# VITA-Group/LightGaussian

Measured on AMD Instinct MI355X. Metric: views/sec fwd+bwd @1080p (N Gaussians), higher is better.
Workload: dtype f32; 1 GPU; 3000000 synthetic Gaussians (SURVEY 8d generator, seed 20250103), 1920x1080, SH degree 3, fwdbwd through gaussian_renderer.render, 200-camera orbit; n_gaussians=3000000, width=1920, height=1080, mode=fwdbwd, views=200, exp=hardware, loss=L1 (HIP, lg_loss_forward/backward with LG_FLAG_L1_ONLY), parallelism=camera-shard x1

## Files before the change

### lightgaussian_amd/csrc/lg_api.hip

```cpp
#include "lg_host.h"
#include "lg_wave.h"
#include "lg_rows.h"
#include "lg_preprocess.h"
#include "lg_binning.h"
#include "lg_blend.h"
#include "lg_loss.h"
#include "lg_prune.h"
#include "lg_knn.h"
#include "lg_compact.h"
#include "lg_vq.h"
#include "lg_vq_train.h"
#include "lg_vq_color.h"
#include "lg_vq_color_bwd.h"
#include "lg_adam.h"
#include "lg_densify.h"
#include "lg_mcmc.h"
#include "lg_features.h"
#include "lg_camera.h"
#include "lg_absgrad.h"
#include "lg_filter3d.h"
#include "lg_normals.h"
#include "lg_distortion.h"
#include "lg_sensitivity.h"
#include "lg_tsdf.h"
// ... 186 lines not shown
    const lg_view* v; const lg_gaussians* g; const Bounded* bounded; lg_alloc_fn alloc; void* alloc_user; int weight_policy;
    float* out_color; int32_t* out_radii; int32_t* out_count; float* out_score; void** binning_out; int64_t* num_rendered;
    hipStream_t stream; bool debug, prof;
    int N, nblk; ViewGeom q; GeomView geo; ImgView img; BinView bin;
    KeyPlan kp; ForwardPlan plan;
    int64_t cap;
    bool k1_cleared_sort;
    PinnedSlot vslot;
    uint32_t* device_status() const { return bounded ? bounded->status : nullptr; }
    int front_end();
    int binning();
    int blend();
    int score();
    int epilogue();
};

int Forward::front_end()
{
    const bool count = out_count != nullptr;
    if (bounded) {
        if (!bounded->binning || bounded->capacity <= 0 || bounded->capacity >= (1ll << 30) || !(bounded->max_depth > 0.2f))
            return fail(LG_ERR_INVALID_ARGUMENT, "lg_forward_bounded: binning buffer, 0 < max_rendered < 2^30 and max_depth > 0.2 required");
        kp = make_key_plan(q.ntiles, N, __builtin_bit_cast(uint32_t, bounded->max_depth), v->flags);
        cap = bounded->capacity;
        bin = carve_bin(bounded->binning, cap, q.W, q.H, q.S);
        if (N == 0) {
            HIP_TRY(lg_zero_async(geo.counters, 16, stream));
            if (bounded->status) HIP_TRY(lg_zero_async(bounded->status, 16, stream));
            HIP_TRY(lg_zero_async(bin.ranges, (size_t)q.ntiles * 8, stream));
        }
    }
    plan = make_forward_plan(v->flags, count, weight_policy, N, bounded ? cap : 1);
    const bool host_words = bounded && bounded->host_status;
    if (host_words) {
        if (!vslot.p) return fail(LG_ERR_ALLOC, "hipHostMalloc of the status slot failed");
        if (N > 0) { vslot.p[1] = vslot.p[2] = vslot.p[3] = 0u; __atomic_store_n(&vslot.p[0], LG_STATUS_PENDING, __ATOMIC_RELEASE); }
        else memset(vslot.p, 0, 16);
    }
    uint32_t* k1_clear = nullptr;
    uint32_t k1_nclear = 0;
    if (bounded && plan.live) {
        k1_clear = (uint32_t*)bin.sort_temp;
        k1_nclear = (uint32_t)(lg_sort_clear_bytes(lg_sort_layout((size_t)cap), (unsigned)kp.sort_passes()) / 4);
    }
    k1_cleared_sort = k1_clear != nullptr;
    if (N > 0) {
        {
            ProfScope ps(prof, "preprocess", stream);
            const bool direct = !(v->flags & LG_FLAG_K1_LDS), raw = v->flags & LG_FLAG_RAW_PARAMS;
            const size_t k1_dyn = (direct && g->shs && !g->colors_precomp && !plan.k1_skip_color) ? LG_K1_PAD_LDS : 0;
            preprocess_kernel(raw, direct, v->flags & LG_FLAG_ANTIALIAS)<<<nblk, LG_PP, k1_dyn, stream>>>(
                N, g->M, v->sh_degree, q.W, q.H, v->tanfovx, v->tanfovy, v->scale_modifier, v->prefiltered, plan.k1_skip_color ? 1 : 0, v->viewmatrix,
                v->projmatrix, v->campos, g->means3D, g->shs, g->shs_rest, g->colors_precomp, g->opacities, g->scales, g->rotations, g->cov3D_precomp, geo,
                out_radii, plan.k1_clears_count ? out_count : nullptr, out_score, k1_clear, k1_nclear, (v->flags & LG_FLAG_SAVE_SH_JACOBIAN) ? 1 : 0);
        }
        KCHECK("lg_preprocess");
        {
            ProfScope ps(prof, "scan", stream);
            lg_scan_blocks<<<(nblk + LG_PART - 1) / LG_PART, LG_PART, 0, stream>>>(nblk, geo.blk_sum, geo.blk_dmax, geo.blk_off, geo.part_sum,
                                                                                  geo.part_dmax, geo.part_prefix, geo.counters + 8,
                                                                                  bounded ? (uint32_t)cap : 0xFFFFFFFFu,
                                                                                  bounded ? kp.depth_bits : 32, geo.counters,
                                                                                  host_words ? vslot.p : device_status());
        }
        KCHECK("lg_scan_blocks");
    }
    if (!bounded) {
        uint32_t h_counters[4] = {0, 0, 0, 0};
        if (N > 0) {
            PinnedSlot slot;
            if (!slot.p) return fail(LG_ERR_ALLOC, "hipHostMalloc of the read-back slot failed");
            HIP_TRY(hipMemcpyAsync(slot.p, geo.counters, 16, hipMemcpyDeviceToHost, stream));
            HIP_TRY(hipStreamSynchronize(stream));
            for (int k = 0; k < 4; k++) h_counters[k] = slot.p[k];
            if (v->prefiltered && h_counters[1]) return fail(LG_ERR_PREFILTERED, "Point is filtered although prefiltered is set. This shouldn't happen!");
            if (h_counters[0] & 1u) return fail(LG_ERR_INVALID_ARGUMENT, "more than 2^32-1 tile instances in one view");
        }
        cap = h_counters[3];
        if (cap >= (1ll << 30)) return fail(LG_ERR_INVALID_ARGUMENT, "more than 2^30-1 tile instances in one view");
        kp = make_key_plan(q.ntiles, N, h_counters[2], v->flags);
        plan = make_forward_plan(v->flags, count, weight_policy, N, cap);
        void* bin_p = alloc(alloc_user, carve_bin(nullptr, cap, q.W, q.H, q.S).total);
        if (!bin_p) return fail(LG_ERR_ALLOC, "binning allocator returned NULL");
        if (binning_out) *binning_out = bin_p;
        bin = carve_bin(bin_p, cap, q.W, q.H, q.S);
        if (num_rendered) *num_rendered = cap;
        if (cap == 0) HIP_TRY(lg_zero_async(bin.ranges, (size_t)q.ntiles * 8, stream));
    }
    g_stats.num_rendered = bounded ? -1 : cap;
    g_stats.num_visible = -1;
    return LG_OK;
}

int Forward::binning()
{
    if (!plan.live) return LG_OK;
    const int sort_begin = kp.sort_begin(), sort_end = kp.sort_end();
    const LgSortLayout SL = lg_sort_layout((size_t)cap);
    if (!k1_cleared_sort) HIP_TRY(lg_zero_async(bin.sort_temp, lg_sort_clear_bytes(SL, (unsigned)kp.sort_passes()), stream));
    uint32_t* hist = (uint32_t*)((char*)bin.sort_temp + SL.hist_off);
    {
        ProfScope ps(prof, "duplicate", stream);
        const int dgrid = std::max(1, std::min((nblk + 4 * LG_DUP_WAVES - 1) / (4 * LG_DUP_WAVES), LG_DUP_GRID));
        lg_duplicate<<<dgrid, LG_DUP_THREADS, 0, stream>>>(N, nblk, q.gx, kp.stored(), kp.store_drop, kp.gid_bits, sort_begin, sort_end, (uint32_t)cap, geo.touched,
                                                          geo.blk_off, geo.part_prefix, geo.counters, geo.offsets, geo.tinfo, bin.keys_in, q.ntiles, bin.ranges, hist,
                                                          kp.two_stage ? 0xFFFFFFFFu : 0u, bin.long_tiles);
    }
// ... 2180 lines not shown
```

### lightgaussian_amd/csrc/lg_binning.h

```cpp
#pragma once

#include "lg_host.h"
#include "lg_wave.h"

#define LG_PART 1024

__global__ void __launch_bounds__(LG_PART)
lg_scan_blocks(int nblk, const uint32_t* __restrict__ blk_sum, const uint32_t* __restrict__ blk_dmax, uint32_t* __restrict__ blk_off,
               uint32_t* part_sum, uint32_t* part_dmax, uint32_t* __restrict__ part_prefix, uint32_t* done, uint32_t capacity,
               int depth_bits, uint32_t* __restrict__ counters, uint32_t* __restrict__ status)
{
    __shared__ uint32_t wsum[16], wmax[16], wflag[16];
    __shared__ uint32_t s_last;
    const uint32_t tid = threadIdx.x, lane = tid & 63u, wave = tid >> 6;
    const int nparts = (int)gridDim.x;
    {
        const int i = (int)blockIdx.x * LG_PART + (int)tid;
        const uint32_t v = i < nblk ? blk_sum[i] : 0u, d = i < nblk ? blk_dmax[i] : 0u;
        const uint32_t inc = lg_wave_scan_incl(v, lane);
        uint32_t m = d & 0x7FFFFFFFu, f = d >> 31;
#pragma unroll
        for (int sh = 32; sh > 0; sh >>= 1) { m = max(m, (uint32_t)__shfl_xor((int)m, sh)); f |= (uint32_t)__shfl_xor((int)f, sh); }
        lg_block_scan_put(wsum, wave, lane, inc);
        if (lane == 63u) { wmax[wave] = m; wflag[wave] = f; }
// ... 63 lines not shown
}

#define LG_DUP_THREADS 1024
#ifndef LG_DUP_GRID
#define LG_DUP_GRID 512
#endif
#define LG_DUP_WAVES (LG_DUP_THREADS / 64)
__global__ void __launch_bounds__(LG_DUP_THREADS)
lg_duplicate(int N, int nblk, int gx, int stored_depth_bits, int store_drop, int gid_bits, int sort_begin, int sort_end, uint32_t capacity,
             const uint32_t* __restrict__ touched, const uint32_t* __restrict__ blk_off, const uint32_t* __restrict__ part_prefix,
             const uint32_t* __restrict__ counters,
             uint32_t* __restrict__ offsets, uint4* __restrict__ tinfo, uint64_t* __restrict__ keys,
             int ntiles, uint2* __restrict__ ranges, uint32_t* __restrict__ hist, uint32_t range_init, uint32_t* __restrict__ long_tiles)
{
    __shared__ uint32_t lh[LG_SORT_MAX_PASSES * 256];
    __shared__ uint32_t s_exc[LG_DUP_WAVES][64], s_xy[LG_DUP_WAVES][64], s_w[LG_DUP_WAVES][64], s_hi[LG_DUP_WAVES][64], s_lo[LG_DUP_WAVES][64];
    const uint32_t tid = threadIdx.x, lane = tid & 63u, wave = tid >> 6;
    for (int t = blockIdx.x * LG_DUP_THREADS + (int)tid; t < ntiles; t += gridDim.x * LG_DUP_THREADS) ranges[t] = make_uint2(range_init, 0u);
    if (blockIdx.x == 0 && tid == 0) long_tiles[0] = 0u;
    const int passes = (sort_end - sort_begin + 7) / 8;
    for (int i = (int)tid; i < passes * 256; i += LG_DUP_THREADS) lh[i] = 0;
    __syncthreads();
    if (counters[0] != 0u) return;
    const int sh = stored_depth_bits + gid_bits;
    const int ngroups = (nblk + 3) / 4;
    for (int g = blockIdx.x * LG_DUP_WAVES + (int)wave; g < ngroups; g += gridDim.x * LG_DUP_WAVES) {
        uint32_t t4[4], base4[4];
        uint4 r4[4];
#pragma unroll
        for (int u = 0; u < 4; u++) {
            const int b = g * 4 + u, i = b * 64 + (int)lane;
            t4[u] = (b < nblk && i < N) ? touched[i] : 0u;
            base4[u] = b < nblk ? blk_off[b] + part_prefix[b / LG_PART] : 0u;
        }
#pragma unroll
        for (int u = 0; u < 4; u++) {
            const int i = (g * 4 + u) * 64 + (int)lane;
            r4[u] = make_uint4(0, 0, 0, 0);
            if (t4[u]) r4[u] = tinfo[i];
        }
#pragma unroll
        for (int u = 0; u < 4; u++) {
            const int b = g * 4 + u, i = b * 64 + (int)lane;
            const uint32_t t = t4[u], base = base4[u];
            const uint4 r = r4[u];
            const uint32_t inc = lg_wave_scan_incl(t, lane);
            const uint32_t total = (uint32_t)__builtin_amdgcn_readlane((int)inc, 63);
            if (b < nblk && i < N) offsets[i] = base + inc;
            if (total != 0u) {
                const uint32_t exc = inc - t;
                if (t) tinfo[i].w = base + exc;
                s_exc[wave][lane] = exc;
                s_xy[wave][lane] = r.x;
                s_w[wave][lane] = (r.y & 0xFFFFu) - (r.x & 0xFFFFu);
                const uint64_t low = ((uint64_t)((r.z - LG_DEPTH_BIAS) >> store_drop) << gid_bits) | (uint32_t)i;
                s_lo[wave][lane] = (uint32_t)low;
                s_hi[wave][lane] = (uint32_t)(low >> 32);
                lg_wave_lds_sync();
                for (uint32_t p = lane; p < total; p += 64u) {
                    uint32_t j = 0;
#pragma unroll
                    for (uint32_t step = 32; step > 0; step >>= 1)
                        if (s_exc[wave][j + step] <= p) j += step;
                    const uint32_t k = p - s_exc[wave][j], w = s_w[wave][j], xy = s_xy[wave][j];
                    const uint32_t ky = k / w, kx = k - ky * w;
                    const uint32_t tile = ((xy >> 16) + ky) * (uint32_t)gx + (xy & 0xFFFFu) + kx;
                    const uint64_t pos = (uint64_t)base + p;
                    const uint64_t key = ((uint64_t)tile << sh) | ((uint64_t)s_hi[wave][j] << 32) | s_lo[wave][j];
                    if (pos < capacity) keys[pos] = key;
                    for (int q = 0; q < passes; q++) {
                        const int bit = sort_begin + 8 * q, nb = min(8, sort_end - bit);
                        atomicAdd(&lh[q * 256 + (uint32_t)((key >> bit) & ((1u << nb) - 1u))], 1u);
                    }
                }
                __builtin_amdgcn_wave_barrier();
            }
        }
    }
    __syncthreads();
    for (int i = (int)tid; i < passes * 256; i += LG_DUP_THREADS)
        if (lh[i]) atomicAdd(&hist[i], lh[i]);
}

__device__ __forceinline__ uint32_t lg_slot_of(const uint4 r, int tx, int ty)
{
    const int x0 = r.x & 0xFFFF, y0 = r.x >> 16, x1 = r.y & 0xFFFF;
    return r.w + (uint32_t)((ty - y0) * (x1 - x0) + (tx - x0));
}

#define LG_RUN_SHORT 32u
__device__ __forceinline__ uint32_t lg_low_bits(uint64_t key, int gid_bits, uint32_t gid_mask, int store_drop, uint32_t low_mask,
                                                const uint4* __restrict__ tinfo)
{
    if (store_drop == 0) return (uint32_t)(key >> gid_bits) & low_mask;
    return (tinfo[(uint32_t)key & gid_mask].z - LG_DEPTH_BIAS) & low_mask;
}

__device__ __forceinline__ void lg_wave_sort_run(uint32_t i, uint32_t e, int low_bits, int gid_bits, uint32_t gid_mask, int store_drop,
                                                 uint64_t* entries, uint64_t* scratch, const uint4* __restrict__ tinfo, uint32_t* cnt ,
                                                 uint32_t lane)
{
    const uint32_t low_mask = low_bits >= 32 ? 0xFFFFFFFFu : ((1u << low_bits) - 1u);
    uint64_t* src = entries;
    uint64_t* dst = scratch;
    for (int shift = 0; shift < low_bits; shift += 8) {
        const uint32_t dmask = (1u << min(8, low_bits - shift)) - 1u;
        for (uint32_t c = lane; c < 256u; c += 64u) cnt[c] = 0u;
        lg_wave_lds_sync();
        for (uint32_t a = i + lane; a < e; a += 64u)
            atomicAdd(&cnt[(lg_low_bits(src[a], gid_bits, gid_mask, store_drop, low_mask, tinfo) >> shift) & dmask], 1u);
        lg_wave_lds_sync();
        {
            const uint32_t c0 = cnt[4u * lane], c1 = cnt[4u * lane + 1u], c2 = cnt[4u * lane + 2u], c3 = cnt[4u * lane + 3u];
            const uint32_t own = c0 + c1 + c2 + c3;
            const uint32_t ex = lg_wave_scan_incl(own, lane) - own;
            cnt[4u * lane] = ex; cnt[4u * lane + 1u] = ex + c0; cnt[4u * lane + 2u] = ex + c0 + c1; cnt[4u * lane + 3u] = ex + c0 + c1 + c2;
        }
        lg_wave_lds_sync();
        for (uint32_t a0 = i; a0 < e; a0 += 64u) {
            const uint32_t a = a0 + lane;
            const bool valid = a < e;
            const uint64_t k = valid ? src[a] : 0ull;
            const uint32_t d = valid ? (lg_low_bits(k, gid_bits, gid_mask, store_drop, low_mask, tinfo) >> shift) & dmask : 0u;
            uint64_t peers = __ballot(valid);
#pragma unroll
            for (int b = 0; b < 8; b++) {
                const bool bit = (d >> b) & 1u;
                const uint64_t m = __ballot(bit);
                peers &= bit ? m : ~m;
            }
            const uint32_t below = prefix_popc(peers);
            uint32_t pos = 0;
            if (valid) pos = cnt[d] + below;
            lg_wave_lds_sync();
            if (valid && below == 0u) cnt[d] += (uint32_t)__popcll(peers);
            lg_wave_lds_sync();
            if (valid) dst[i + pos] = k;
        }
        __threadfence();
        uint64_t* t = src; src = dst; dst = t;
// ... 483 lines not shown
```

### lightgaussian_amd/csrc/lg_math.h

```cpp
#pragma once
#include <math.h>
#include <stddef.h>
#include <stdint.h>

#if defined(__HIPCC__)
#define LG_HD __host__ __device__ __forceinline__
#else
#define LG_HD static inline
#endif

#define LG_TILE 16
#define LG_ALPHA_MIN (1.0f / 255.0f)
#define LG_T_MIN 0.0001f
#define LG_ALPHA_MAX 0.99f

enum { LG_W_ONE = 0, LG_W_OPACITY = 1, LG_W_ALPHA = 2, LG_W_ALPHA_T = 3 };

LG_HD float lg_bits2f(uint32_t u) { union { uint32_t u; float f; } c; c.u = u; return c.f; }
LG_HD uint32_t lg_f2bits(float f) { union { uint32_t u; float f; } c; c.f = f; return c.u; }

LG_HD float lg_exp(float x)
{
    x = fmaxf(x, -87.0f);
    float t = x * 1.44269504088896341f;
// ... 110 lines not shown
    float b = o.U[0] * T2[3] + o.U[1] * T2[4] + o.U[2] * T2[5];
    float c = o.V[0] * T2[3] + o.V[1] * T2[4] + o.V[2] * T2[5];
    o.a = a + 0.3f; o.b = b; o.c = c + 0.3f;
    o.a0 = a; o.c0 = c;
}

#define LG_AA_FLOOR 0.000025f
LG_HD float lg_aa_ratio(float a0, float b, float c0, float a, float c)
{
    const float det0 = a0 * c0 - b * b;
    const float det1 = a * c - b * b;
    return det0 / det1;
}
LG_HD float lg_aa_rho(float x) { return sqrtf(fmaxf(LG_AA_FLOOR, x)); }
LG_HD float lg_aa_backward(float a0, float b, float c0, float a, float c, float op, float gp, float& dL_da, float& dL_db, float& dL_dc)
{
    const float det0 = a0 * c0 - b * b;
    const float det1 = a * c - b * b;
    const float x = det0 / det1;
    const float rho = lg_aa_rho(x);
    if (x > LG_AA_FLOOR) {
        const float gx = (op * gp) * 0.5f / rho;
        const float s = gx / (det1 * det1);
        const float bb = b * b;
        dL_da += s * (0.3f * (c0 * c + bb));
        dL_dc += s * (0.3f * (a0 * a + bb));
        dL_db += s * (-2.0f * b * (0.3f * (a0 + c0) + 0.09f));
    }
    return rho;
}

LG_HD void lg_view_point(const float* vm, float px, float py, float pz, float& vx, float& vy, float& vz)
{
    vx = vm[0] * px + vm[4] * py + vm[8] * pz + vm[12];
    vy = vm[1] * px + vm[5] * py + vm[9] * pz + vm[13];
    vz = vm[2] * px + vm[6] * py + vm[10] * pz + vm[14];
}
LG_HD void lg_hom_point(const float* pm, float px, float py, float pz, float& hx, float& hy, float& m_w)
{
    hx = pm[0] * px + pm[4] * py + pm[8] * pz + pm[12];
    hy = pm[1] * px + pm[5] * py + pm[9] * pz + pm[13];
    const float hw = pm[3] * px + pm[7] * py + pm[11] * pz + pm[15];
    m_w = 1.0f / (hw + 0.0000001f);
}
LG_HD void lg_focal(int W, int H, float tanfovx, float tanfovy, float& fx, float& fy)
{
    fx = (float)W / (2.0f * tanfovx); fy = (float)H / (2.0f * tanfovy);
}

struct LgSplat {
    float x, y, depth;
    float ha, nb, hc;
    float hx, hy;
    int radius;
    int rx0, ry0, rx1, ry1;
    int tx0, ty0, tx1, ty1;
};

template <bool AA>
LG_HD bool lg_project_t(const float* vm, const float* pm, float px, float py, float pz, const float* cov3D, float opacity,
                        int W, int H, float tanfovx, float tanfovy, LgSplat& o, float& op_out)
{
    float vx, vy, vz;
    lg_view_point(vm, px, py, pz, vx, vy, vz);
    if (vz <= 0.2f) return false;
    float hxm = pm[0] * px + pm[4] * py + pm[8] * pz + pm[12];
    float hym = pm[1] * px + pm[5] * py + pm[9] * pz + pm[13];
    float hwm = pm[3] * px + pm[7] * py + pm[11] * pz + pm[15];
    float p_w = 1.0f / (hwm + 0.0000001f);
    float ndcx = hxm * p_w, ndcy = hym * p_w;

    float fx, fy;
    lg_focal(W, H, tanfovx, tanfovy, fx, fy);
    LgEwa e;
    lg_ewa(vm, vx, vy, vz, fx, fy, 1.3f * tanfovx, 1.3f * tanfovy, e);
    LgCov2D c2;
    lg_cov2d(e.T2, cov3D, c2);
    const float a = c2.a, b = c2.b, c = c2.c;
    float det = a * c - b * b;
    if (det == 0.0f) return false;
    if (AA) { opacity = opacity * lg_aa_rho(lg_aa_ratio(c2.a0, b, c2.c0, a, c)); op_out = opacity; }
    float det_inv = 1.0f / det;
    float A = c * det_inv, B = -b * det_inv, C = a * det_inv;
    float mid = 0.5f * (a + c);
    float sq = sqrtf(fmaxf(0.1f, mid * mid - det));
    float l1 = mid + sq, l2 = mid - sq;
    float rad = ceilf(3.0f * sqrtf(fmaxf(l1, l2)));
    float ix = ((ndcx + 1.0f) * (float)W - 1.0f) * 0.5f;
    float iy = ((ndcy + 1.0f) * (float)H - 1.0f) * 0.5f;
    const int gx = (W + LG_TILE - 1) / LG_TILE, gy = (H + LG_TILE - 1) / LG_TILE;
    const float big = 1.0e7f;
    int r0 = (int)fminf(big, fmaxf(-big, (ix - rad) / (float)LG_TILE));
    int r1 = (int)fminf(big, fmaxf(-big, (iy - rad) / (float)LG_TILE));
    int r2 = (int)fminf(big, fmaxf(-big, (ix + rad + (float)(LG_TILE - 1)) / (float)LG_TILE));
    int r3 = (int)fminf(big, fmaxf(-big, (iy + rad + (float)(LG_TILE - 1)) / (float)LG_TILE));
    o.rx0 = r0 < 0 ? 0 : (r0 > gx ? gx : r0);
    o.ry0 = r1 < 0 ? 0 : (r1 > gy ? gy : r1);
    o.rx1 = r2 < 0 ? 0 : (r2 > gx ? gx : r2);
    o.ry1 = r3 < 0 ? 0 : (r3 > gy ? gy : r3);
    if ((o.rx1 - o.rx0) * (o.ry1 - o.ry0) == 0) return false;
    o.x = ix; o.y = iy; o.depth = vz; o.radius = (int)rad;
    o.ha = -0.5f * A; o.nb = -B; o.hc = -0.5f * C;

    o.tx0 = o.rx0; o.ty0 = o.ry0; o.tx1 = o.rx1; o.ty1 = o.ry1;
    o.hx = INFINITY; o.hy = INFINITY;
    if (!(opacity >= LG_ALPHA_MIN)) {
        if (opacity < LG_ALPHA_MIN) { o.tx1 = o.tx0; o.ty1 = o.ty0; o.hx = -1.0f; o.hy = -1.0f; }
        return true;
    }
    float amp = (a * c) / det;
    if (amp > 0.0f && amp < 100.0f && rad < 4096.0f) {
        float dmax = rad + (float)LG_TILE;
        float smax = (fabsf(o.ha) + fabsf(o.nb) + fabsf(o.hc)) * dmax * dmax;
        float tau = logf(opacity * 255.0f);
        float taup = (tau + 1.0e-6f * smax) * 1.00001f + 1.0e-4f;
        if (taup < 1.0e30f) {
            float hx = sqrtf(2.0f * taup * a) * 1.001f + 0.01f;
            float hy = sqrtf(2.0f * taup * c) * 1.001f + 0.01f;
            int t0 = (int)fminf(big, fmaxf(-big, ceilf((ix - hx - (float)(LG_TILE - 1)) / (float)LG_TILE)));
            int t1 = (int)fminf(big, fmaxf(-big, floorf((ix + hx) / (float)LG_TILE))) + 1;
            int u0 = (int)fminf(big, fmaxf(-big, ceilf((iy - hy - (float)(LG_TILE - 1)) / (float)LG_TILE)));
            int u1 = (int)fminf(big, fmaxf(-big, floorf((iy + hy) / (float)LG_TILE))) + 1;
            o.tx0 = t0 > o.rx0 ? t0 : o.rx0; o.tx1 = t1 < o.rx1 ? t1 : o.rx1;
            o.ty0 = u0 > o.ry0 ? u0 : o.ry0; o.ty1 = u1 < o.ry1 ? u1 : o.ry1;
            if (o.tx0 > o.rx1) o.tx0 = o.rx1;
            if (o.ty0 > o.ry1) o.ty0 = o.ry1;
            if (o.tx1 < o.tx0) o.tx1 = o.tx0;
            if (o.ty1 < o.ty0) o.ty1 = o.ty0;
            o.hx = hx; o.hy = hy;
        }
    }
    return true;
}
LG_HD bool lg_project(const float* vm, const float* pm, float px, float py, float pz, const float* cov3D, float opacity,
                      int W, int H, float tanfovx, float tanfovy, LgSplat& o)
{
    float unused;
    return lg_project_t<false>(vm, pm, px, py, pz, cov3D, opacity, W, H, tanfovx, tanfovy, o, unused);
}

#define LG_SH_C0 0.28209479177387814f
#define LG_SH_C1 0.4886025119029199f
#define LG_SH_C2_0 1.0925484305920792f
#define LG_SH_C2_1 -1.0925484305920792f
#define LG_SH_C2_2 0.31539156525252005f
#define LG_SH_C2_3 -1.0925484305920792f
#define LG_SH_C2_4 0.5462742152960396f
#define LG_SH_C3_0 -0.5900435899266435f
#define LG_SH_C3_1 2.890611442640554f
#define LG_SH_C3_2 -0.4570457994644658f
#define LG_SH_C3_3 0.3731763325901154f
#define LG_SH_C3_4 -0.4570457994644658f
#define LG_SH_C3_5 1.445305721320277f
#define LG_SH_C3_6 -0.5900435899266435f

LG_HD void lg_sh_to_rgb(int deg, const float* sh, float px, float py, float pz, const float* campos, float rgb[3],
                        uint32_t& clamp_bits)
{
    float dx = px - campos[0], dy = py - campos[1], dz = pz - campos[2];
    float len = sqrtf(dx * dx + dy * dy + dz * dz);
    dx = dx / len; dy = dy / len; dz = dz / len;
    clamp_bits = 0;
    for (int c = 0; c < 3; c++) {
        float res = LG_SH_C0 * sh[0 * 3 + c];
        if (deg > 0) {
            res = res - LG_SH_C1 * dy * sh[1 * 3 + c] + LG_SH_C1 * dz * sh[2 * 3 + c] - LG_SH_C1 * dx * sh[3 * 3 + c];
            if (deg > 1) {
                float xx = dx * dx, yy = dy * dy, zz = dz * dz, xy = dx * dy, yz = dy * dz, xz = dx * dz;
                res = res + LG_SH_C2_0 * xy * sh[4 * 3 + c] + LG_SH_C2_1 * yz * sh[5 * 3 + c] +
                      LG_SH_C2_2 * (2.0f * zz - xx - yy) * sh[6 * 3 + c] + LG_SH_C2_3 * xz * sh[7 * 3 + c] +
                      LG_SH_C2_4 * (xx - yy) * sh[8 * 3 + c];
                if (deg > 2) {
                    res = res + LG_SH_C3_0 * dy * (3.0f * xx - yy) * sh[9 * 3 + c] + LG_SH_C3_1 * xy * dz * sh[10 * 3 + c] +
                          LG_SH_C3_2 * dy * (4.0f * zz - xx - yy) * sh[11 * 3 + c] +
                          LG_SH_C3_3 * dz * (2.0f * zz - 3.0f * xx - 3.0f * yy) * sh[12 * 3 + c] +
                          LG_SH_C3_4 * dx * (4.0f * zz - xx - yy) * sh[13 * 3 + c] +
                          LG_SH_C3_5 * dz * (xx - yy) * sh[14 * 3 + c] + LG_SH_C3_6 * dx * (xx - 3.0f * yy) * sh[15 * 3 + c];
                }
            }
        }
        float v = res + 0.5f;
        if (v < 0.0f) clamp_bits |= (1u << c);
        rgb[c] = fmaxf(v, 0.0f);
    }
}

LG_HD float lg_pair_power(float gx, float gy, float ha, float nb, float hc, float pxf, float pyf, float& dx, float& dy)
{
    dx = gx - pxf; dy = gy - pyf;
    return fmaf(fmaf(ha, dx, nb * dy), dx, (hc * dy) * dy);
}
// ... 943 lines not shown
```

### lightgaussian_amd/csrc/lg_plan.h

```cpp
#pragma once
#include <stdint.h>
#include <algorithm>
#include "../../include/lightgaussian.h"
#include "../../include/lightgaussian_score.h"

static inline int bits_for(uint32_t n)
{
    int b = 0;
    while (b < 32 && (1ull << b) < n) b++;
    return b;
}
static inline int lg_gid_bits(int N) { return bits_for((uint32_t)(N > 1 ? N : 2)); }
static inline uint32_t lg_gid_mask(int gid_bits) { return gid_bits >= 32 ? 0xFFFFFFFFu : ((1u << gid_bits) - 1u); }

#define LG_DEPTH_BIAS (124u << 23)
#define LG_NARROW_KEY_BITS 40
struct KeyPlan {
    int tile_bits, gid_bits, depth_bits;
    int store_drop;
    bool two_stage;
    uint32_t gid_mask;
    int stored() const { return depth_bits - store_drop; }
    int tile_shift() const { return gid_bits + stored(); }
    int sort_begin() const { return two_stage ? tile_shift() : gid_bits; }
    int sort_end() const { return tile_shift() + (tile_bits > 0 ? tile_bits : 1); }
    int sort_passes() const { return (sort_end() - sort_begin() + 7) / 8; }
};
static inline KeyPlan make_key_plan(int ntiles, int N, uint32_t dmax_bits, uint32_t flags)
{
    KeyPlan k;
    k.tile_bits = bits_for((uint32_t)ntiles);
    k.gid_bits = lg_gid_bits(N);
    const uint32_t dspan = dmax_bits > LG_DEPTH_BIAS ? dmax_bits - LG_DEPTH_BIAS : 0u;
    k.depth_bits = bits_for(dspan + 1u) > 0 ? bits_for(dspan + 1u) : 1;
    const int avail = (flags & LG_FLAG_NARROW_KEY) ? LG_NARROW_KEY_BITS : 64;
    k.store_drop = std::max(0, std::min(k.depth_bits - 1, k.tile_bits + k.depth_bits + k.gid_bits - avail));
    k.two_stage = !(flags & LG_FLAG_SORT_ALL_BITS);
    k.gid_mask = lg_gid_mask(k.gid_bits);
    return k;
}

enum { LG_CHAIN_NONE = 0, LG_CHAIN_COLOR = 1, LG_CHAIN_COUNT = 2 };
enum { LG_SCORE_NONE = 0, LG_SCORE_COUNT = 1, LG_SCORE_COUNT_OPACITY = 2, LG_SCORE_SLOTS = 3, LG_SCORE_SLOTS_MAX = 4 };
constexpr bool lg_blend_merges(int fscore, bool color) { return fscore != 0 && !color; }
struct ForwardPlan {
    bool live;
    bool count;
    bool exact;
    bool color;
    int fscore;
    bool fmax;
    bool merge;
    bool clear_slots;
    bool k1_skip_color;
    bool k1_clears_count;
    int long_mode;
    int long_chain;
// ... 32 lines not shown
```

### lightgaussian_amd/csrc/lg_preprocess.h

```cpp
#pragma once

#include "lg_host.h"
#include "lg_wave.h"
#include "lg_rows.h"

#define LG_PP 64
#define LG_ID_BITS 29
#define LG_ID_MASK ((1u << LG_ID_BITS) - 1u)
#define LG_SH_MAXF 48
#ifndef LG_K1_PAD_LDS
#define LG_K1_PAD_LDS 7900
#endif
#ifndef LG_K9_GATHER
#define LG_K9_GATHER 4
#endif
#define LG_COOP_ROWS 48u

__device__ __forceinline__ void stage_sh_rows(const float* __restrict__ shs, int i0, int rows, int rowf, uint64_t need_mask,
                                              float* lds, uint32_t lane)
{
    const float* src = shs + (size_t)i0 * rowf;
    const int nfl = rows * rowf;
    const bool vec_ok = ((reinterpret_cast<uintptr_t>(src) & 15u) == 0);
    if (vec_ok) {
        const int nvec = nfl >> 2;
        for (int q = (int)lane; q < nvec; q += LG_PP) {
            const int f = q << 2;
            if ((rowf & 3) == 0 && !((need_mask >> (f / rowf)) & 1ull)) continue;
            *reinterpret_cast<float4*>(lds + f) = *reinterpret_cast<const float4*>(src + f);
        }
        for (int f = (nvec << 2) + (int)lane; f < nfl; f += LG_PP) lds[f] = src[f];
    } else {
        for (int f = (int)lane; f < nfl; f += LG_PP) lds[f] = src[f];
    }
}

struct __attribute__((packed, aligned(4))) lg_f4u { float x, y, z, w; };
template <int K0>
__device__ __forceinline__ void read_row_direct(const float* __restrict__ row, int nfl, float* sh )
{
#pragma unroll
    for (int q = 0; q < (LG_SH_MAXF - K0 + 3) / 4; q++) {
        float v[4] = {0.0f, 0.0f, 0.0f, 0.0f};
        if (4 * q + 4 <= nfl) {
            const lg_f4u t = reinterpret_cast<const lg_f4u*>(row)[q];
            v[0] = t.x; v[1] = t.y; v[2] = t.z; v[3] = t.w;
        } else {
#pragma unroll
            for (int c = 0; c < 4; c++)
                if (4 * q + c < nfl) v[c] = row[4 * q + c];
        }
#pragma unroll
        for (int c = 0; c < 4; c++)
            if (K0 + 4 * q + c < LG_SH_MAXF) sh[K0 + 4 * q + c] = v[c];
    }
}
__device__ __forceinline__ float lg_sigmoid(float x) { return 1.0f / (1.0f + expf(-x)); }

template <bool RAW, bool DIRECT, bool AA>
#ifdef LG_K1_WAVES
__global__ void __launch_bounds__(LG_PP) __attribute__((amdgpu_waves_per_eu(LG_K1_WAVES, 8)))
#else
__global__ void __launch_bounds__(LG_PP)
#endif
lg_preprocess(int N, int M, int D, int W, int H, float tanfovx, float tanfovy, float mod, int prefiltered, int skip_color,
              const float* __restrict__ viewmatrix, const float* __restrict__ projmatrix, const float* __restrict__ campos,
              const float* __restrict__ means3D, const float* __restrict__ shs, const float* __restrict__ shs_rest,
              const float* __restrict__ colors_precomp,
              const float* __restrict__ opacities, const float* __restrict__ scales, const float* __restrict__ rotations,
              const float* __restrict__ cov3D_precomp, GeomView g, int32_t* __restrict__ radii, int32_t* __restrict__ zero_count,
              float* __restrict__ zero_score, uint32_t* __restrict__ clear_words, uint32_t n_clear, int save_jac)
{
    __shared__ __attribute__((aligned(16))) float sh_rows[DIRECT ? 4 : LG_PP * LG_SH_MAXF];
    __shared__ float4 st_rec[LG_PP * 3];
    __shared__ __attribute__((aligned(16))) float st_jac[LG_PP * 9];
    static_assert(LG_REC_F4 == 3, "coalesced record store assumes packed 48-byte records");
    const uint32_t lane = threadIdx.x;
    const int i0 = blockIdx.x * LG_PP;
    const int i = i0 + (int)lane;
    for (uint32_t w = blockIdx.x * LG_PP + lane; w < n_clear; w += gridDim.x * LG_PP) clear_words[w] = 0u;
    float vm[16], pm[16], cp[3];
#pragma unroll
    for (int k = 0; k < 16; k++) { vm[k] = viewmatrix[k]; pm[k] = projmatrix[k]; }
    cp[0] = campos[0]; cp[1] = campos[1]; cp[2] = campos[2];
    bool vis = false, violation = false;
    float px = 0, py = 0, pz = 0, op = 0, op_aa = 0;
    float cov[6] = {0, 0, 0, 0, 0, 0};
    LgSplat sp;
    if (i < N) {
        px = means3D[3 * (size_t)i]; py = means3D[3 * (size_t)i + 1]; pz = means3D[3 * (size_t)i + 2];
        const float vz = vm[2] * px + vm[6] * py + vm[10] * pz + vm[14];
        if (vz > 0.2f) {
            if (cov3D_precomp) {
#pragma unroll
                for (int k = 0; k < 6; k++) cov[k] = cov3D_precomp[6 * (size_t)i + k];
            } else {
                float sc[3] = { scales[3 * (size_t)i], scales[3 * (size_t)i + 1], scales[3 * (size_t)i + 2] };
                const float4 q4 = *reinterpret_cast<const float4*>(rotations + 4 * (size_t)i);
                float q[4] = { q4.x, q4.y, q4.z, q4.w };
                if (RAW) {
                    sc[0] = expf(sc[0]); sc[1] = expf(sc[1]); sc[2] = expf(sc[2]);
                    const float qn = fmaxf(sqrtf((q[0] * q[0] + q[1] * q[1]) + (q[2] * q[2] + q[3] * q[3])), 1e-12f);
                    q[0] /= qn; q[1] /= qn; q[2] /= qn; q[3] /= qn;
                }
                lg_cov3d(sc, mod, q, cov);
            }
            op = RAW ? lg_sigmoid(opacities[i]) : opacities[i];
            vis = lg_project_t<AA>(vm, pm, px, py, pz, cov, op, W, H, tanfovx, tanfovy, sp, op_aa);
        } else if (prefiltered) {
            violation = true;
        }
        if (zero_count) { zero_count[i] = 0; zero_score[i] = 0.0f; }
    }
    const uint64_t vmask = __ballot(vis);
    const bool split = RAW && shs_rest != nullptr;
    const int rowf = split ? 3 * (M - 1) : 3 * M;
    if (!DIRECT && !skip_color && shs && vmask && rowf > 0) {
        stage_sh_rows(split ? shs_rest : shs, i0, min(LG_PP, N - i0), rowf, vmask, sh_rows, lane);
        lg_wave_lds_sync();
    }
    uint32_t touched = 0;
    if (i < N) {
        int radius = 0;
        if (vis) {
            radius = sp.radius;
            touched = (uint32_t)((sp.tx1 - sp.tx0) * (sp.ty1 - sp.ty0));
            float rgb[3] = {0.0f, 0.0f, 0.0f};
            uint32_t cb = 0;
            if (skip_color) {
            } else if (colors_precomp) {
                rgb[0] = colors_precomp[3 * (size_t)i]; rgb[1] = colors_precomp[3 * (size_t)i + 1]; rgb[2] = colors_precomp[3 * (size_t)i + 2];
            } else {
                float sh[LG_SH_MAXF];
                const float* row = DIRECT ? shs + (size_t)i * rowf : sh_rows + lane * rowf;
                const int nact = (D + 1) * (D + 1) * 3;
                if (split && DIRECT) {
                    sh[0] = shs[3 * (size_t)i]; sh[1] = shs[3 * (size_t)i + 1]; sh[2] = shs[3 * (size_t)i + 2];
                    read_row_direct<3>(shs_rest + (size_t)i * rowf, nact - 3, sh);
                } else if (DIRECT) {
                    read_row_direct<0>(row, nact, sh);
                } else if (split) {
                    sh[0] = shs[3 * (size_t)i]; sh[1] = shs[3 * (size_t)i + 1]; sh[2] = shs[3 * (size_t)i + 2];
#pragma unroll
                    for (int k = 3; k < LG_SH_MAXF; k++) sh[k] = (k < nact) ? row[k - 3] : 0.0f;
                } else if ((rowf & 3) == 0) {
#pragma unroll
                    for (int q = 0; q < LG_SH_MAXF / 4; q++) {
                        float4 v4 = make_float4(0, 0, 0, 0);
                        if (q * 4 < nact) v4 = reinterpret_cast<const float4*>(row)[q];
                        sh[4 * q] = v4.x; sh[4 * q + 1] = v4.y; sh[4 * q + 2] = v4.z; sh[4 * q + 3] = v4.w;
                    }
                } else {
#pragma unroll
                    for (int k = 0; k < LG_SH_MAXF; k++) sh[k] = (k < nact) ? row[k] : 0.0f;
                }
                lg_sh_to_rgb(D, sh, px, py, pz, cp, rgb, cb);
                if (save_jac) {
                    float J[9];
                    lg_sh_dir_jacobian(D, sh, px, py, pz, cp, J);
#pragma unroll
                    for (int k = 0; k < 9; k++) st_jac[9 * lane + k] = J[k];
                }
            }
            st_rec[3 * lane + 0] = make_float4(sp.x, sp.y, sp.ha, sp.nb);
            st_rec[3 * lane + 1] = make_float4(sp.hc, AA ? op_aa : op, rgb[0], rgb[1]);
            st_rec[3 * lane + 2] = make_float4(rgb[2], sp.hx, sp.hy, __uint_as_float((uint32_t)i | (cb << LG_ID_BITS)));
            g.tinfo[i] = make_uint4((uint32_t)sp.tx0 | ((uint32_t)sp.ty0 << 16), (uint32_t)sp.tx1 | ((uint32_t)sp.ty1 << 16),
                                    __float_as_uint(sp.depth), 0u);
        }
        radii[i] = radius;
        g.visible[i] = radius > 0 ? (uint8_t)1 : (uint8_t)0;
        g.touched[i] = touched;
    }
    if (vmask) {
        lg_wave_lds_sync();
        const int nrec = min(LG_PP, N - i0);
#pragma unroll
        for (int k = 0; k < 3; k++)
            if ((int)(k * LG_PP + lane) < 3 * nrec) g.rec[3 * (size_t)i0 + k * LG_PP + lane] = st_rec[k * LG_PP + lane];
        if (save_jac && shs && !skip_color) {
            float* dstj = g.shjac + 9 * (size_t)i0;
            const int nfl = 9 * nrec, nvec = nfl >> 2;
            for (int q = (int)lane; q < nvec; q += LG_PP) reinterpret_cast<float4*>(dstj)[q] = reinterpret_cast<const float4*>(st_jac)[q];
            for (int f = (nvec << 2) + (int)lane; f < nfl; f += LG_PP) dstj[f] = st_jac[f];
        }
    }
    const uint32_t dmax = lg_wave_all_max(vis ? __float_as_uint(sp.depth) : 0u);
    uint32_t tsum = touched;
#pragma unroll
    for (int sh = 32; sh > 0; sh >>= 1) tsum += (uint32_t)__shfl_xor((int)tsum, sh);
    const uint64_t any_violation = __ballot(violation);
    if (lane == 0) {
        g.blk_dmax[blockIdx.x] = dmax | (any_violation ? 0x80000000u : 0u);
        g.blk_sum[blockIdx.x] = tsum;
        if (blockIdx.x == 0) {
            g.counters[8] = 0u;
            g.counters[9] = (save_jac && shs && !skip_color) ? LG_SHJAC_MAGIC : 0u;
        }
    }
}


__device__ __forceinline__ bool lg_k9_view_has_rows(const uint32_t* counters, const uint32_t* meta, uint32_t S, bool marker)
{
    return counters[0] == 0u && meta[2] == S && (!marker || counters[9] == LG_SHJAC_MAGIC);
}

__device__ __forceinline__ void lg_k9_gather_coop(const float4* part, uint32_t my_t, uint32_t my_u0, uint32_t lane, float (&coop)[9])
{
#pragma unroll
    for (int k9 = 0; k9 < 9; k9++) coop[k9] = 0.0f;
    uint64_t big = __ballot(my_t > LG_COOP_ROWS);
    while (big) {
        const int src = (int)__builtin_ctzll(big);
        big &= big - 1;
        const uint32_t t = (uint32_t)__builtin_amdgcn_readlane((int)my_t, src);
        const uint32_t u0 = (uint32_t)__builtin_amdgcn_readlane((int)my_u0, src);
        float acc9[9] = {0, 0, 0, 0, 0, 0, 0, 0, 0};
        for (uint32_t u = u0 + lane; u < u0 + t; u += LG_PP) {
            const float4* rp = part + 3 * (size_t)u;
// ... 315 lines not shown
```

### lightgaussian_amd/rasterizer.py

```python
import ctypes as C
import threading
from typing import NamedTuple

import torch
import torch.nn as nn

from . import _lib


class GaussianRasterizationSettings(NamedTuple):
    image_height: int
    image_width: int
    tanfovx: float
    tanfovy: float
    bg: torch.Tensor
    scale_modifier: float
    viewmatrix: torch.Tensor
    projmatrix: torch.Tensor
    sh_degree: int
    campos: torch.Tensor
    prefiltered: bool
    debug: bool
    f_count: bool = False


_OPTIONS = {"weight_policy": _lib.WEIGHT_OPACITY, "fast_exp": True, "profile": False, "skip_color_in_count": False,
            "fuse_getters": True, "sync_free": "validated", "max_depth": 100.0, "capacity_margin": 1.25,
            "segment_length": 0, "long_tiles": "auto", "count_long_tiles": "serial", "camera_grad": False, "antialiasing": False,
            "filter_3d": True, "absgrad": False, "score_reduce": "sum",
            "sh_jacobian": True, "narrow_key": False, "sort_all_bits": False, "k1_lds": False, "count_wide_band": False}
_PER_CALL_ONLY = ("pending", "tag", "status_override", "differentiated", "sh_grad_sink", "score_out", "count_sum")
_LONG_TILES = ("serial", "auto", "parallel")
_STRICT_BOOL = ("camera_grad", "antialiasing", "filter_3d", "absgrad")
_tls = threading.local()


SCORE_REDUCTIONS = ("sum", "max")
FLAG_SCORE_MAX = 65536
WEIGHT_POLICIES = {"one": _lib.WEIGHT_ONE, "opacity": _lib.WEIGHT_OPACITY, "alpha": _lib.WEIGHT_ALPHA, "alpha_t": _lib.WEIGHT_ALPHA_T}


def weight_policy_id(value):
    if isinstance(value, str):
        if value.lower() not in WEIGHT_POLICIES:
            raise ValueError(f"weight_policy must be one of {tuple(WEIGHT_POLICIES)} (or a _lib.WEIGHT_* number)")
        return WEIGHT_POLICIES[value.lower()]
    if int(value) not in WEIGHT_POLICIES.values():
        raise ValueError(f"weight_policy {value!r}: not a _lib.WEIGHT_* value")
    return int(value)


def score_reduce_name(value):
    if not isinstance(value, str) or value.lower() not in SCORE_REDUCTIONS:
        raise ValueError(f"score_reduce must be one of {SCORE_REDUCTIONS}")
    return value.lower()


def check_score_reduce(score_reduce, weight_policy):
    name = score_reduce_name(score_reduce)
    if name == "max" and weight_policy_id(weight_policy) not in (_lib.WEIGHT_ALPHA, _lib.WEIGHT_ALPHA_T):
        raise ValueError('score_reduce="max" needs weight_policy "alpha" or "alpha_t" (every hit of "one" / "opacity" adds the same value)')
    return name


def _validate(name, value):
    if name == "weight_policy":
        weight_policy_id(value)
    if name == "score_reduce":
        score_reduce_name(value)
    if name == "long_tiles" and value not in _LONG_TILES:
        raise ValueError(f"long_tiles must be one of {_LONG_TILES}")
    if name == "count_long_tiles" and value not in ("serial", "parallel"):
        raise ValueError("count_long_tiles must be 'serial' or 'parallel'")
    if name in _STRICT_BOOL and not isinstance(value, bool):
        raise ValueError(f"{name} must be True or False")
    if name == "segment_length" and (int(value) < 0 or (int(value) != 0 and (int(value) < 64 or int(value) % 64))):
        raise ValueError("segment_length must be 0 (library default, 512) or a multiple of 64")


def _check_options(kw):
    for k, v in kw.items():
        if k not in _OPTIONS and k not in _PER_CALL_ONLY:
            raise KeyError(k)
        _validate(k, v)


def set_option(name, value):
    if name not in _OPTIONS:
        raise KeyError(name)
    _validate(name, value)
    prev = _OPTIONS[name]
# ... 69 lines not shown
    return t


class _Call:

    def __init__(self, rs, means3D, sh, colors_precomp, opacities, scales, rotations, cov3D_precomp, exact, sh_rest=None, raw=False, opts=None,
                 differentiated=False):
        opts = opts if opts is not None else resolve_options()
        self.opts = opts
        dev = means3D.device
        if dev.type != "cuda":
            raise RuntimeError("lightgaussian_amd rasterizer needs tensors on a HIP device (torch 'cuda'); there is no CPU path")
        self.dev = dev
        self.means3D = _prep(means3D, dev)
        self.sh = _prep(sh, dev)
        self.colors = _prep(colors_precomp, dev)
        self.opac = _prep(opacities, dev)
        self.scales = _prep(scales, dev)
        self.rots = _prep(rotations, dev)
        self.cov = _prep(cov3D_precomp, dev)
        self.bg = _prep(rs.bg, dev)
        self.vm = _prep(rs.viewmatrix, dev)
        self.pm = _prep(rs.projmatrix, dev)
        self.cp = _prep(rs.campos, dev)
        self.sh_rest = _prep(sh_rest, dev)
        N = self.means3D.shape[0] if self.means3D is not None else 0
        M = 0 if self.sh is None else int(self.sh.shape[1]) + (0 if sh_rest is None else int(sh_rest.shape[1]))
        flags = _lib.FLAG_RAW_PARAMS if raw else 0
        if differentiated and opts["sh_jacobian"]:
            flags |= _lib.FLAG_SAVE_SH_JACOBIAN
        if rs.debug:
            flags |= _lib.FLAG_DEBUG
        if opts["fast_exp"] and not exact:
            flags |= _lib.FLAG_FAST_EXP
        flags |= _lib.profile_flag(opts["profile"])
        if exact and opts["skip_color_in_count"]:
            flags |= _lib.FLAG_SKIP_COLOR
        if exact and check_score_reduce(opts.get("score_reduce", "sum"), opts["weight_policy"]) == "max":
            flags |= FLAG_SCORE_MAX
        if exact:
            flags |= _lib.FLAG_LONG_PARALLEL if opts["count_long_tiles"] == "parallel" else _lib.FLAG_LONG_SERIAL
        else:
            flags |= {"serial": _lib.FLAG_LONG_SERIAL, "auto": 0, "parallel": _lib.FLAG_LONG_PARALLEL}[opts["long_tiles"]]
        if opts["narrow_key"]:
            flags |= _lib.FLAG_NARROW_KEY
        if opts["sort_all_bits"]:
            flags |= _lib.FLAG_SORT_ALL_BITS
        if opts["k1_lds"]:
            flags |= _lib.FLAG_K1_LDS
        if opts["count_wide_band"]:
            flags |= _lib.FLAG_COUNT_WIDE_BAND
        if opts["antialiasing"]:
            flags |= _lib.FLAG_ANTIALIAS
        if opts.get("absgrad") and not exact:
            flags |= _lib.FLAG_ABSGRAD
        self.view = _lib.lg_view(int(rs.image_height), int(rs.image_width), float(rs.tanfovx), float(rs.tanfovy),
                                 _lib.ptr(self.bg), float(rs.scale_modifier), _lib.ptr(self.vm), _lib.ptr(self.pm),
                                 int(rs.sh_degree), _lib.ptr(self.cp), int(bool(rs.prefiltered)), flags, int(opts["segment_length"]))
        self.g = _lib.lg_gaussians(N, M, _lib.ptr(self.means3D), _lib.ptr(self.sh), _lib.ptr(self.colors), _lib.ptr(self.opac),
                                   _lib.ptr(self.scales), _lib.ptr(self.rots), _lib.ptr(self.cov), _lib.ptr(self.sh_rest))
        self.N, self.M = N, M


def _bare_view(rs, flags, segment_length):
    return _lib.lg_view(int(rs.image_height), int(rs.image_width), float(rs.tanfovx), float(rs.tanfovy), None, float(rs.scale_modifier),
                        None, None, int(rs.sh_degree), None, 0, int(flags), int(segment_length))


_CAP_LOCK = threading.Lock()
_CAPACITY = {}


class PendingBatch:

    def __init__(self):
        self.items = []
        self.lock = threading.Lock()

    def add(self, status, key, tag):
        with self.lock:
            self.items.append((status, key, tag))

    def __len__(self):
        return len(self.items)

    def drop_oldest(self, n):
        with self.lock:
            del self.items[:n]

    def resolve(self, capacity_margin=None):
        margin = float(capacity_margin if capacity_margin is not None else resolve_options()["capacity_margin"])
        with self.lock:
            pend, self.items = self.items, []
        if not pend:
            return []
        live = [p[0] for p in pend if p[0] is not None]
        it = iter(torch.stack([t.to(live[0].device) for t in live]).cpu().tolist() if live else [])
        out = []
        for st, key, tag in pend:
            if st is None:
                out.append((tag, False))
                continue
            flags, _viol, _dmax, R = next(it)
            flags &= 0xFFFFFFFF
            R &= 0xFFFFFFFF
            out.append((tag, flags != 0))
# ... 376 lines not shown
```

Baseline: 670.8 views/s.

## Add per-splat tile occupancy mask to skip tiles the ellipse cannot reach

For splats covering a small rectangle of tiles (at most 16, both sides at least 2), preprocessing evaluates the Gaussian's quadratic form at the nearest point of each tile and builds a bitmask of tiles that can exceed the alpha threshold. The mask is packed into the upper bits of tinfo.y, the touched count becomes its popcount, and duplication and slot lookup map through mask-select and popcount. This is meant to cut sort keys, sort work and per-tile blending on empty corner tiles. In exchange it adds per-splat arithmetic in preprocessing and overloads the upper bits of tinfo.y, which any other reader of ty1 would now misread.

```diff
diff --git a/include/lightgaussian_tilemask.h b/include/lightgaussian_tilemask.h
--- /dev/null
+++ b/include/lightgaussian_tilemask.h
@@ -0,0 +1,6 @@
+#ifndef LIGHTGAUSSIAN_TILEMASK_H
+#define LIGHTGAUSSIAN_TILEMASK_H
+
+enum { LG_FLAG_TILE_MASK = 131072 };
+
+#endif
diff --git a/lightgaussian_amd/csrc/lg_api.hip b/lightgaussian_amd/csrc/lg_api.hip
--- a/lightgaussian_amd/csrc/lg_api.hip
+++ b/lightgaussian_amd/csrc/lg_api.hip
@@ -262,7 +262,8 @@
             preprocess_kernel(raw, direct, v->flags & LG_FLAG_ANTIALIAS)<<<nblk, LG_PP, k1_dyn, stream>>>(
                 N, g->M, v->sh_degree, q.W, q.H, v->tanfovx, v->tanfovy, v->scale_modifier, v->prefiltered, plan.k1_skip_color ? 1 : 0, v->viewmatrix,
                 v->projmatrix, v->campos, g->means3D, g->shs, g->shs_rest, g->colors_precomp, g->opacities, g->scales, g->rotations, g->cov3D_precomp, geo,
-                out_radii, plan.k1_clears_count ? out_count : nullptr, out_score, k1_clear, k1_nclear, (v->flags & LG_FLAG_SAVE_SH_JACOBIAN) ? 1 : 0);
+                out_radii, plan.k1_clears_count ? out_count : nullptr, out_score, k1_clear, k1_nclear, (v->flags & LG_FLAG_SAVE_SH_JACOBIAN) ? 1 : 0,
+                (v->flags & LG_FLAG_TILE_MASK) ? 1 : 0);
         }
         KCHECK("lg_preprocess");
         {
diff --git a/lightgaussian_amd/csrc/lg_binning.h b/lightgaussian_amd/csrc/lg_binning.h
--- a/lightgaussian_amd/csrc/lg_binning.h
+++ b/lightgaussian_amd/csrc/lg_binning.h
@@ -139,7 +139,7 @@
                 if (t) tinfo[i].w = base + exc;
                 s_exc[wave][lane] = exc;
                 s_xy[wave][lane] = r.x;
-                s_w[wave][lane] = (r.y & 0xFFFFu) - (r.x & 0xFFFFu);
+                s_w[wave][lane] = ((r.y & 0xFFFFu) - (r.x & 0xFFFFu)) | (r.y & 0xFFFF0000u);
                 const uint64_t low = ((uint64_t)((r.z - LG_DEPTH_BIAS) >> store_drop) << gid_bits) | (uint32_t)i;
                 s_lo[wave][lane] = (uint32_t)low;
                 s_hi[wave][lane] = (uint32_t)(low >> 32);
@@ -149,7 +149,8 @@
 #pragma unroll
                     for (uint32_t step = 32; step > 0; step >>= 1)
                         if (s_exc[wave][j + step] <= p) j += step;
-                    const uint32_t k = p - s_exc[wave][j], w = s_w[wave][j], xy = s_xy[wave][j];
+                    const uint32_t wm = s_w[wave][j], w = wm & 0xFFFFu, xy = s_xy[wave][j];
+                    const uint32_t k = lg_rect_tile(wm >> 16, p - s_exc[wave][j]);
                     const uint32_t ky = k / w, kx = k - ky * w;
                     const uint32_t tile = ((xy >> 16) + ky) * (uint32_t)gx + (xy & 0xFFFFu) + kx;
                     const uint64_t pos = (uint64_t)base + p;
@@ -171,8 +172,7 @@
 
 __device__ __forceinline__ uint32_t lg_slot_of(const uint4 r, int tx, int ty)
 {
-    const int x0 = r.x & 0xFFFF, y0 = r.x >> 16, x1 = r.y & 0xFFFF;
-    return r.w + (uint32_t)((ty - y0) * (x1 - x0) + (tx - x0));
+    return r.w + lg_rect_slot(r.x, r.y, tx, ty);
 }
 
 #define LG_RUN_SHORT 32u
diff --git a/lightgaussian_amd/csrc/lg_math.h b/lightgaussian_amd/csrc/lg_math.h
--- a/lightgaussian_amd/csrc/lg_math.h
+++ b/lightgaussian_amd/csrc/lg_math.h
@@ -186,6 +186,7 @@
     float x, y, depth;
     float ha, nb, hc;
     float hx, hy;
+    float taup, smax;
     int radius;
     int rx0, ry0, rx1, ry1;
     int tx0, ty0, tx1, ty1;
@@ -237,7 +238,7 @@
     o.ha = -0.5f * A; o.nb = -B; o.hc = -0.5f * C;
 
     o.tx0 = o.rx0; o.ty0 = o.ry0; o.tx1 = o.rx1; o.ty1 = o.ry1;
-    o.hx = INFINITY; o.hy = INFINITY;
+    o.hx = INFINITY; o.hy = INFINITY; o.taup = INFINITY; o.smax = 0.0f;
     if (!(opacity >= LG_ALPHA_MIN)) {
         if (opacity < LG_ALPHA_MIN) { o.tx1 = o.tx0; o.ty1 = o.ty0; o.hx = -1.0f; o.hy = -1.0f; }
         return true;
@@ -261,7 +262,7 @@
             if (o.ty0 > o.ry1) o.ty0 = o.ry1;
             if (o.tx1 < o.tx0) o.tx1 = o.tx0;
             if (o.ty1 < o.ty0) o.ty1 = o.ty0;
-            o.hx = hx; o.hy = hy;
+            o.hx = hx; o.hy = hy; o.taup = taup; o.smax = smax;
         }
     }
     return true;
@@ -271,6 +272,53 @@
 {
     float unused;
     return lg_project_t<false>(vm, pm, px, py, pz, cov3D, opacity, W, H, tanfovx, tanfovy, o, unused);
+}
+
+#define LG_TILE_MASKED 0x10000u
+LG_HD uint32_t lg_tile_mask(const LgSplat& s)
+{
+    const int w = s.tx1 - s.tx0, h = s.ty1 - s.ty0;
+    if (!(s.taup < 1.0e30f) || w < 2 || h < 2 || w * h > 16) return 0u;
+    const float thr = -(s.taup + 1.0e-6f * s.smax);
+    const float iha = 0.5f / s.ha, ihc = 0.5f / s.hc;
+    uint32_t mask = 0u, bit = 1u;
+    for (int ty = s.ty0; ty < s.ty1; ty++) {
+        const float ylo = (float)(ty * LG_TILE) - s.y, yhi = (float)(ty * LG_TILE + (LG_TILE - 1)) - s.y;
+        const float dye = fminf(fmaxf(0.0f, ylo), yhi);
+        for (int tx = s.tx0; tx < s.tx1; tx++, bit <<= 1) {
+            const float xlo = (float)(tx * LG_TILE) - s.x, xhi = (float)(tx * LG_TILE + (LG_TILE - 1)) - s.x;
+            const float dxe = fminf(fmaxf(0.0f, xlo), xhi);
+            const float dy1 = fminf(fmaxf(-(s.nb * dxe) * ihc, ylo), yhi);
+            const float p1 = (s.ha * dxe + s.nb * dy1) * dxe + (s.hc * dy1) * dy1;
+            const float dx2 = fminf(fmaxf(-(s.nb * dye) * iha, xlo), xhi);
+            const float p2 = (s.ha * dx2 + s.nb * dye) * dx2 + (s.hc * dye) * dye;
+            if (!(p1 < thr) || !(p2 < thr)) mask |= bit;
+        }
+    }
+    if (mask == (1u << (w * h)) - 1u) return 0u;
+    return mask | LG_TILE_MASKED;
+}
+LG_HD uint32_t lg_tile_count(const LgSplat& s, uint32_t m)
+{
+    return m ? (uint32_t)__builtin_popcount(m & 0xFFFFu) : (uint32_t)((s.tx1 - s.tx0) * (s.ty1 - s.ty0));
+}
+LG_HD uint32_t lg_mask_select(uint32_t mask, uint32_t p)
+{
+    uint32_t k = 0u, c = (uint32_t)__builtin_popcount(mask & 0xFFu);
+    if (p >= c) { p -= c; k = 8u; mask >>= 8; }
+    c = (uint32_t)__builtin_popcount(mask & 0xFu);
+    if (p >= c) { p -= c; k += 4u; mask >>= 4; }
+    c = (uint32_t)__builtin_popcount(mask & 0x3u);
+    if (p >= c) { p -= c; k += 2u; mask >>= 2; }
+    if (p >= (mask & 1u)) k += 1u;
+    return k;
+}
+LG_HD uint32_t lg_rect_tile(uint32_t mask, uint32_t p) { return mask ? lg_mask_select(mask, p) : p; }
+LG_HD uint32_t lg_rect_slot(uint32_t rx, uint32_t ry, int tx, int ty)
+{
+    const int x0 = (int)(rx & 0xFFFFu), y0 = (int)(rx >> 16), x1 = (int)(ry & 0xFFFFu);
+    const uint32_t k = (uint32_t)((ty - y0) * (x1 - x0) + (tx - x0)), mask = ry >> 16;
+    return mask ? (uint32_t)__builtin_popcount(mask & ((1u << (k & 15u)) - 1u)) : k;
 }
 
 #define LG_SH_C0 0.28209479177387814f
diff --git a/lightgaussian_amd/csrc/lg_plan.h b/lightgaussian_amd/csrc/lg_plan.h
--- a/lightgaussian_amd/csrc/lg_plan.h
+++ b/lightgaussian_amd/csrc/lg_plan.h
@@ -3,6 +3,7 @@
 #include <algorithm>
 #include "../../include/lightgaussian.h"
 #include "../../include/lightgaussian_score.h"
+#include "../../include/lightgaussian_tilemask.h"
 
 static inline int bits_for(uint32_t n)
 {
diff --git a/lightgaussian_amd/csrc/lg_preprocess.h b/lightgaussian_amd/csrc/lg_preprocess.h
--- a/lightgaussian_amd/csrc/lg_preprocess.h
+++ b/lightgaussian_amd/csrc/lg_preprocess.h
@@ -69,7 +69,7 @@
               const float* __restrict__ colors_precomp,
               const float* __restrict__ opacities, const float* __restrict__ scales, const float* __restrict__ rotations,
               const float* __restrict__ cov3D_precomp, GeomView g, int32_t* __restrict__ radii, int32_t* __restrict__ zero_count,
-              float* __restrict__ zero_score, uint32_t* __restrict__ clear_words, uint32_t n_clear, int save_jac)
+              float* __restrict__ zero_score, uint32_t* __restrict__ clear_words, uint32_t n_clear, int save_jac, int tile_mask)
 {
     __shared__ __attribute__((aligned(16))) float sh_rows[DIRECT ? 4 : LG_PP * LG_SH_MAXF];
     __shared__ float4 st_rec[LG_PP * 3];
@@ -124,11 +124,13 @@
         int radius = 0;
         if (vis) {
             radius = sp.radius;
-            touched = (uint32_t)((sp.tx1 - sp.tx0) * (sp.ty1 - sp.ty0));
+            uint32_t tmask = 0u;
             float rgb[3] = {0.0f, 0.0f, 0.0f};
             uint32_t cb = 0;
             if (skip_color) {
+                if (tile_mask) tmask = lg_tile_mask(sp);
             } else if (colors_precomp) {
+                if (tile_mask) tmask = lg_tile_mask(sp);
                 rgb[0] = colors_precomp[3 * (size_t)i]; rgb[1] = colors_precomp[3 * (size_t)i + 1]; rgb[2] = colors_precomp[3 * (size_t)i + 2];
             } else {
                 float sh[LG_SH_MAXF];
@@ -154,6 +156,7 @@
 #pragma unroll
                     for (int k = 0; k < LG_SH_MAXF; k++) sh[k] = (k < nact) ? row[k] : 0.0f;
                 }
+                if (tile_mask) tmask = lg_tile_mask(sp);
                 lg_sh_to_rgb(D, sh, px, py, pz, cp, rgb, cb);
                 if (save_jac) {
                     float J[9];
@@ -165,7 +168,8 @@
             st_rec[3 * lane + 0] = make_float4(sp.x, sp.y, sp.ha, sp.nb);
             st_rec[3 * lane + 1] = make_float4(sp.hc, AA ? op_aa : op, rgb[0], rgb[1]);
             st_rec[3 * lane + 2] = make_float4(rgb[2], sp.hx, sp.hy, __uint_as_float((uint32_t)i | (cb << LG_ID_BITS)));
-            g.tinfo[i] = make_uint4((uint32_t)sp.tx0 | ((uint32_t)sp.ty0 << 16), (uint32_t)sp.tx1 | ((uint32_t)sp.ty1 << 16),
+            touched = lg_tile_count(sp, tmask);
+            g.tinfo[i] = make_uint4((uint32_t)sp.tx0 | ((uint32_t)sp.ty0 << 16), (uint32_t)sp.tx1 | (tmask << 16),
                                     __float_as_uint(sp.depth), 0u);
         }
         radii[i] = radius;
diff --git a/lightgaussian_amd/rasterizer.py b/lightgaussian_amd/rasterizer.py
--- a/lightgaussian_amd/rasterizer.py
+++ b/lightgaussian_amd/rasterizer.py
@@ -27,16 +27,17 @@
 _OPTIONS = {"weight_policy": _lib.WEIGHT_OPACITY, "fast_exp": True, "profile": False, "skip_color_in_count": False,
             "fuse_getters": True, "sync_free": "validated", "max_depth": 100.0, "capacity_margin": 1.25,
             "segment_length": 0, "long_tiles": "auto", "count_long_tiles": "serial", "camera_grad": False, "antialiasing": False,
-            "filter_3d": True, "absgrad": False, "score_reduce": "sum",
+            "filter_3d": True, "absgrad": False, "score_reduce": "sum", "tile_mask": True,
             "sh_jacobian": True, "narrow_key": False, "sort_all_bits": False, "k1_lds": False, "count_wide_band": False}
 _PER_CALL_ONLY = ("pending", "tag", "status_override", "differentiated", "sh_grad_sink", "score_out", "count_sum")
 _LONG_TILES = ("serial", "auto", "parallel")
-_STRICT_BOOL = ("camera_grad", "antialiasing", "filter_3d", "absgrad")
+_STRICT_BOOL = ("camera_grad", "antialiasing", "filter_3d", "absgrad", "tile_mask")
 _tls = threading.local()
 
 
 SCORE_REDUCTIONS = ("sum", "max")
 FLAG_SCORE_MAX = 65536
+FLAG_TILE_MASK = 131072
 WEIGHT_POLICIES = {"one": _lib.WEIGHT_ONE, "opacity": _lib.WEIGHT_OPACITY, "alpha": _lib.WEIGHT_ALPHA, "alpha_t": _lib.WEIGHT_ALPHA_T}
 
 
@@ -212,6 +213,8 @@
             flags |= _lib.FLAG_COUNT_WIDE_BAND
         if opts["antialiasing"]:
             flags |= _lib.FLAG_ANTIALIAS
+        if opts.get("tile_mask"):
+            flags |= FLAG_TILE_MASK
         if opts.get("absgrad") and not exact:
             flags |= _lib.FLAG_ABSGRAD
         self.view = _lib.lg_view(int(rs.image_height), int(rs.image_width), float(rs.tanfovx), float(rs.tanfovy),
```

After: 677.2 views/s (median of 6 runs). No clear change (+1.0%).
